# VisionDepth/VisionDepth3D

Hardware: NVIDIA H100
Metric: end-to-end frames/sec (depth+stereo) (higher is better)
Workload: dtype f16 GEMM operands, fp32 accumulate; DIBR fp32

## Files before the change

visiondepth3d_b200/csrc/umma_attention.cuh:

```cuda
#pragma once
#include "umma_gemm.cuh"

namespace vd3d {

struct AttnArgs {
  int ntok;
  int dmodel;
  __half* out;
  int heads;
  int npad;
};

constexpr int kAttnThreads = 384;
constexpr int kAttnKS = 2;
constexpr int kAttnSmem = 16384  + kAttnKS * (16384  + 16384 ) + 1024  + 256 ;

namespace umma {
__device__ __forceinline__ float quad_max(float x) {
  x = fmaxf(x, __shfl_xor_sync(0xffffffffu, x, 1));
  return fmaxf(x, __shfl_xor_sync(0xffffffffu, x, 2));
}
__device__ __forceinline__ float quad_sum(float x) {
  x += __shfl_xor_sync(0xffffffffu, x, 1);
  return x + __shfl_xor_sync(0xffffffffu, x, 2);
}
__device__ __forceinline__ uint32_t pack_h2(float a, float b) {
  __half2 h = __floats2half2_rn(a, b);
  return *(uint32_t*)&h;
}
}

__global__ void __launch_bounds__(kAttnThreads, 1)
k_umma_attention(const __grid_constant__ CUtensorMap tmQ, const __grid_constant__ CUtensorMap tmK,
                 const __grid_constant__ CUtensorMap tmV, const AttnArgs g) {
  extern __shared__ uint8_t smem_raw[];
  const uint32_t sm = (umma::smem_u32(smem_raw) + 1023u) & ~1023u;
  const uint32_t sQ = sm, sK = sm + 16384, sV = sK + kAttnKS * 16384;
  const uint32_t bars = sV + kAttnKS * 16384;
  const uint32_t q_full = bars, kv_full = bars + 8, kv_empty = kv_full + 8 * kAttnKS;

  const int warp = threadIdx.x >> 5, lane = threadIdx.x & 31;
  const int qblk = blockIdx.x, zq = blockIdx.y, h = zq % g.heads, img = zq / g.heads;
  const int T = (g.ntok + 127) / 128;

  if (warp == 0 && lane == 0) {
    umma::prefetch_tmap(&tmQ);
    umma::prefetch_tmap(&tmK);
    umma::prefetch_tmap(&tmV);
    umma::mbar_init(q_full, 1);
    for (int i = 0; i < kAttnKS; ++i) {
      umma::mbar_init(kv_full + 8 * i, 1);
      umma::mbar_init(kv_empty + 8 * i, 2);
    }
    umma::fence_barrier_init();
  }
  __syncthreads();

  if (warp < 4) {
    if (warp == 0 && lane == 0) {
      umma::mbar_expect_tx(q_full, 16384);
      umma::tma_load_3d(sQ, &tmQ, q_full, 0, qblk * 128, zq);
      for (int t = 0; t < T; ++t) {
        const int ks = t % kAttnKS;
        umma::mbar_wait(kv_empty + 8 * ks, ((t / kAttnKS) & 1) ^ 1);
        const uint32_t fb = kv_full + 8 * ks;
        umma::mbar_expect_tx(fb, 32768);
        umma::tma_load_3d(sK + ks * 16384, &tmK, fb, 0, t * 128, zq);
        const uint32_t dst = sV + ks * 16384;
        umma::tma_load_3d(dst, &tmV, fb, t * 128, 0, zq);
        umma::tma_load_3d(dst + 8192, &tmV, fb, t * 128 + 64, 0, zq);
      }
    }
    return;
  }

  const int wg = (warp >> 2) - 1;
  const int wq = warp & 3;
  const float L2E = 1.4426950408889634f;
  const int cq = 2 * (lane & 3);
  float o[32];
#pragma unroll
  for (int i = 0; i < 32; ++i) o[i] = 0.f;
  float m_run[2] = {-INFINITY, -INFINITY}, l_run[2] = {0.f, 0.f};

  umma::mbar_wait(q_full, 0);
  const uint64_t dq = umma::make_desc(sQ + (uint32_t)(wg * 64 * 128));
  for (int t = 0; t < T; ++t) {
    const int ks = t % kAttnKS;
    umma::mbar_wait(kv_full + 8 * ks, (t / kAttnKS) & 1);
    float s[64];
    {
      const uint64_t dk = umma::make_desc(sK + ks * 16384);
      umma::wgmma_fence();
#pragma unroll
      for (int k = 0; k < 4; ++k) umma::wgmma_m64n128_ss(s, dq + (uint64_t)(2 * k), dk + (uint64_t)(2 * k), k ? 1u : 0u);
      umma::wgmma_commit();
      umma::wgmma_wait<0>();
      umma::fence_regs(s);
    }
    const int nvalid = g.ntok - t * 128;
    float mx[2] = {-INFINITY, -INFINITY};
#pragma unroll
    for (int j = 0; j < 16; ++j)
#pragma unroll
      for (int i = 0; i < 4; ++i) {
        if (nvalid < 128 && 8 * j + cq + (i & 1) >= nvalid) s[4 * j + i] = -INFINITY;
        mx[i >> 1] = fmaxf(mx[i >> 1], s[4 * j + i]);
      }
    float scale[2], mref[2];
#pragma unroll
    for (int rr = 0; rr < 2; ++rr) {
      const float m_new = fmaxf(m_run[rr], umma::quad_max(mx[rr]) * L2E);
      scale[rr] = umma::ex2_fast(m_run[rr] - m_new);
      m_run[rr] = m_new;
      mref[rr] = m_new - 8.0f;
    }
    float ls[2] = {0.f, 0.f};
    uint32_t p[32];
#pragma unroll
    for (int j = 0; j < 16; ++j) {
      const float p0 = umma::ex2_fast(fmaf(s[4 * j + 0], L2E, -mref[0]));
      const float p1 = umma::ex2_fast(fmaf(s[4 * j + 1], L2E, -mref[0]));
      const float p2 = umma::ex2_fast(fmaf(s[4 * j + 2], L2E, -mref[1]));
      const float p3 = umma::ex2_fast(fmaf(s[4 * j + 3], L2E, -mref[1]));
      p[2 * j] = umma::pack_h2(p0, p1);
      p[2 * j + 1] = umma::pack_h2(p2, p3);
      const float2 h0 = __half22float2(*(const __half2*)&p[2 * j]), h1 = __half22float2(*(const __half2*)&p[2 * j + 1]);
      ls[0] += h0.x + h0.y;
      ls[1] += h1.x + h1.y;
    }
#pragma unroll
    for (int rr = 0; rr < 2; ++rr) l_run[rr] = l_run[rr] * scale[rr] + ls[rr];
#pragma unroll
    for (int j = 0; j < 8; ++j) {
      o[4 * j + 0] *= scale[0];
      o[4 * j + 1] *= scale[0];
      o[4 * j + 2] *= scale[1];
      o[4 * j + 3] *= scale[1];
    }
    umma::fence_regs(o);
    umma::wgmma_fence();
#pragma unroll
    for (int kk = 0; kk < 8; ++kk) {
      const uint32_t a[4] = {p[4 * kk], p[4 * kk + 1], p[4 * kk + 2], p[4 * kk + 3]};
      const uint64_t db = umma::make_desc(sV + ks * 16384 + (kk >> 2) * 8192) + (uint64_t)(2 * (kk & 3));
      umma::wgmma_m64n64_rs(o, a, db, 1u);
    }
    umma::wgmma_commit();
    umma::wgmma_wait<0>();
    umma::fence_regs(o);
    if ((threadIdx.x & 127) == 0) umma::mbar_arrive(kv_empty + 8 * ks);
  }

  float inv[2];
#pragma unroll
  for (int rr = 0; rr < 2; ++rr) inv[rr] = 1.0f / umma::quad_sum(l_run[rr]);
  const int r0 = qblk * 128 + wg * 64 + wq * 16 + (lane >> 2);
#pragma unroll
  for (int rr = 0; rr < 2; ++rr) {
    const int m = r0 + 8 * rr;
    if (m >= g.ntok) continue;
    __half* dst = g.out + ((size_t)img * g.npad + m) * g.dmodel + h * 64 + cq;
#pragma unroll
    for (int j = 0; j < 8; ++j)
      *(uint32_t*)(dst + 8 * j) = umma::pack_h2(o[4 * j + 2 * rr] * inv[rr], o[4 * j + 2 * rr + 1] * inv[rr]);
  }
}

}
```

Baseline: 320.3.

## Pipeline FA3-style attention with split K/V barriers, ping-pong warpgroups, and register reallocation

```diff
diff --git a/visiondepth3d_b200/csrc/umma_attention.cuh b/visiondepth3d_b200/csrc/umma_attention.cuh
--- a/visiondepth3d_b200/csrc/umma_attention.cuh
+++ b/visiondepth3d_b200/csrc/umma_attention.cuh
@@ -1,4 +1,6 @@
 #pragma once
+#include <type_traits>
+
 #include "umma_gemm.cuh"
 
 namespace vd3d {
@@ -12,8 +14,11 @@
 };
 
 constexpr int kAttnThreads = 384;
-constexpr int kAttnKS = 2;
+constexpr int kAttnKS = 3;
 constexpr int kAttnSmem = 16384  + kAttnKS * (16384  + 16384 ) + 1024  + 256 ;
+constexpr int kAttnProducerRegs = 24;
+constexpr int kAttnConsumerRegs = 240;
+static_assert(128 * kAttnProducerRegs + 256 * kAttnConsumerRegs <= 65536, "register file overcommitted");
 
 namespace umma {
 __device__ __forceinline__ float quad_max(float x) {
@@ -27,6 +32,87 @@
 __device__ __forceinline__ uint32_t pack_h2(float a, float b) {
   __half2 h = __floats2half2_rn(a, b);
   return *(uint32_t*)&h;
+}
+template <int R>
+__device__ __forceinline__ void fence_regs(uint32_t (&d)[R]) {
+#pragma unroll
+  for (int i = 0; i < R; ++i) asm volatile("" : "+r"(d[i])::"memory");
+}
+__device__ __forceinline__ void bar_sync_256(int id) { asm volatile("bar.sync %0, 256;" ::"r"(id) : "memory"); }
+__device__ __forceinline__ void bar_arrive_256(int id) { asm volatile("bar.arrive %0, 256;" ::"r"(id) : "memory"); }
+
+template <bool kMasked>
+__device__ __forceinline__ void attn_softmax(float (&s)[64], int nvalid, int cq, float (&m_run)[2], float (&scale)[2]) {
+  const float L2E = 1.4426950408889634f;
+  if constexpr (kMasked) {
+#pragma unroll
+    for (int j = 0; j < 16; ++j)
+#pragma unroll
+      for (int i = 0; i < 4; ++i)
+        if (8 * j + cq + (i & 1) >= nvalid) s[4 * j + i] = -INFINITY;
+  }
+  float mx[2];
+#pragma unroll
+  for (int rr = 0; rr < 2; ++rr) {
+    float m[16];
+#pragma unroll
+    for (int j = 0; j < 16; ++j) m[j] = fmaxf(s[4 * j + 2 * rr], s[4 * j + 2 * rr + 1]);
+#pragma unroll
+    for (int j = 0; j < 8; ++j) m[j] = fmaxf(m[j], m[j + 8]);
+#pragma unroll
+    for (int j = 0; j < 4; ++j) m[j] = fmaxf(m[j], m[j + 4]);
+    mx[rr] = fmaxf(fmaxf(m[0], m[2]), fmaxf(m[1], m[3]));
+  }
+  float mref[2];
+#pragma unroll
+  for (int rr = 0; rr < 2; ++rr) {
+    const float m_new = fmaxf(m_run[rr], quad_max(mx[rr]) * L2E);
+    scale[rr] = ex2_fast(m_run[rr] - m_new);
+    m_run[rr] = m_new;
+    mref[rr] = m_new - 8.0f;
+  }
+#pragma unroll
+  for (int j = 0; j < 16; ++j)
+#pragma unroll
+    for (int i = 0; i < 4; ++i) s[4 * j + i] = ex2_fast(fmaf(s[4 * j + i], L2E, -mref[i >> 1]));
+}
+
+__device__ __forceinline__ void attn_pack(const float (&s)[64], uint32_t (&p)[32], float (&o)[32], float (&l_run)[2],
+                                          const float (&scale)[2]) {
+  float ls[2] = {0.f, 0.f};
+#pragma unroll
+  for (int j = 0; j < 16; ++j) {
+    p[2 * j] = pack_h2(s[4 * j + 0], s[4 * j + 1]);
+    p[2 * j + 1] = pack_h2(s[4 * j + 2], s[4 * j + 3]);
+    const float2 h0 = __half22float2(*(const __half2*)&p[2 * j]), h1 = __half22float2(*(const __half2*)&p[2 * j + 1]);
+    ls[0] += h0.x + h0.y;
+    ls[1] += h1.x + h1.y;
+  }
+#pragma unroll
+  for (int rr = 0; rr < 2; ++rr) l_run[rr] = l_run[rr] * scale[rr] + ls[rr];
+#pragma unroll
+  for (int j = 0; j < 8; ++j) {
+    o[4 * j + 0] *= scale[0];
+    o[4 * j + 1] *= scale[0];
+    o[4 * j + 2] *= scale[1];
+    o[4 * j + 3] *= scale[1];
+  }
+}
+
+__device__ __forceinline__ void attn_qk(float (&s)[64], uint64_t dq, uint32_t k_tile) {
+  const uint64_t dk = make_desc(k_tile);
+#pragma unroll
+  for (int k = 0; k < 4; ++k) wgmma_m64n128_ss(s, dq + (uint64_t)(2 * k), dk + (uint64_t)(2 * k), k ? 1u : 0u);
+  wgmma_commit();
+}
+__device__ __forceinline__ void attn_pv(float (&o)[32], const uint32_t (&p)[32], uint32_t v_tile) {
+#pragma unroll
+  for (int kk = 0; kk < 8; ++kk) {
+    const uint32_t a[4] = {p[4 * kk], p[4 * kk + 1], p[4 * kk + 2], p[4 * kk + 3]};
+    const uint64_t db = make_desc(v_tile + (kk >> 2) * 8192) + (uint64_t)(2 * (kk & 3));
+    wgmma_m64n64_rs(o, a, db, 1u);
+  }
+  wgmma_commit();
 }
 }
 
@@ -37,7 +123,8 @@
   const uint32_t sm = (umma::smem_u32(smem_raw) + 1023u) & ~1023u;
   const uint32_t sQ = sm, sK = sm + 16384, sV = sK + kAttnKS * 16384;
   const uint32_t bars = sV + kAttnKS * 16384;
-  const uint32_t q_full = bars, kv_full = bars + 8, kv_empty = kv_full + 8 * kAttnKS;
+  const uint32_t q_full = bars, k_full = bars + 8, k_empty = k_full + 8 * kAttnKS;
+  const uint32_t v_full = k_empty + 8 * kAttnKS, v_empty = v_full + 8 * kAttnKS;
 
   const int warp = threadIdx.x >> 5, lane = threadIdx.x & 31;
   const int qblk = blockIdx.x, zq = blockIdx.y, h = zq % g.heads, img = zq / g.heads;
@@ -49,107 +136,96 @@
     umma::prefetch_tmap(&tmV);
     umma::mbar_init(q_full, 1);
     for (int i = 0; i < kAttnKS; ++i) {
-      umma::mbar_init(kv_full + 8 * i, 1);
-      umma::mbar_init(kv_empty + 8 * i, 2);
+      umma::mbar_init(k_full + 8 * i, 1);
+      umma::mbar_init(k_empty + 8 * i, 2);
+      umma::mbar_init(v_full + 8 * i, 1);
+      umma::mbar_init(v_empty + 8 * i, 2);
     }
     umma::fence_barrier_init();
   }
   __syncthreads();
 
   if (warp < 4) {
+    asm volatile("setmaxnreg.dec.sync.aligned.u32 %0;" ::"n"(kAttnProducerRegs));
     if (warp == 0 && lane == 0) {
       umma::mbar_expect_tx(q_full, 16384);
       umma::tma_load_3d(sQ, &tmQ, q_full, 0, qblk * 128, zq);
       for (int t = 0; t < T; ++t) {
         const int ks = t % kAttnKS;
-        umma::mbar_wait(kv_empty + 8 * ks, ((t / kAttnKS) & 1) ^ 1);
-        const uint32_t fb = kv_full + 8 * ks;
-        umma::mbar_expect_tx(fb, 32768);
-        umma::tma_load_3d(sK + ks * 16384, &tmK, fb, 0, t * 128, zq);
-        const uint32_t dst = sV + ks * 16384;
-        umma::tma_load_3d(dst, &tmV, fb, t * 128, 0, zq);
-        umma::tma_load_3d(dst + 8192, &tmV, fb, t * 128 + 64, 0, zq);
+        const uint32_t ph = ((t / kAttnKS) & 1) ^ 1;
+        umma::mbar_wait(k_empty + 8 * ks, ph);
+        umma::mbar_expect_tx(k_full + 8 * ks, 16384);
+        umma::tma_load_3d(sK + ks * 16384, &tmK, k_full + 8 * ks, 0, t * 128, zq);
+        umma::mbar_wait(v_empty + 8 * ks, ph);
+        const uint32_t vb = v_full + 8 * ks, dst = sV + ks * 16384;
+        umma::mbar_expect_tx(vb, 16384);
+        umma::tma_load_3d(dst, &tmV, vb, t * 128, 0, zq);
+        umma::tma_load_3d(dst + 8192, &tmV, vb, t * 128 + 64, 0, zq);
       }
     }
     return;
   }
+  asm volatile("setmaxnreg.inc.sync.aligned.u32 %0;" ::"n"(kAttnConsumerRegs));
 
   const int wg = (warp >> 2) - 1;
   const int wq = warp & 3;
-  const float L2E = 1.4426950408889634f;
   const int cq = 2 * (lane & 3);
+  const bool lead = (threadIdx.x & 127) == 0;
   float o[32];
 #pragma unroll
   for (int i = 0; i < 32; ++i) o[i] = 0.f;
-  float m_run[2] = {-INFINITY, -INFINITY}, l_run[2] = {0.f, 0.f};
+  float m_run[2] = {-INFINITY, -INFINITY}, l_run[2] = {0.f, 0.f}, scale[2];
+  float s[64];
+  uint32_t p[32];
+
+  if (wg == 1) umma::bar_arrive_256(1);
 
   umma::mbar_wait(q_full, 0);
   const uint64_t dq = umma::make_desc(sQ + (uint32_t)(wg * 64 * 128));
-  for (int t = 0; t < T; ++t) {
-    const int ks = t % kAttnKS;
-    umma::mbar_wait(kv_full + 8 * ks, (t / kAttnKS) & 1);
-    float s[64];
-    {
-      const uint64_t dk = umma::make_desc(sK + ks * 16384);
-      umma::wgmma_fence();
-#pragma unroll
-      for (int k = 0; k < 4; ++k) umma::wgmma_m64n128_ss(s, dq + (uint64_t)(2 * k), dk + (uint64_t)(2 * k), k ? 1u : 0u);
-      umma::wgmma_commit();
-      umma::wgmma_wait<0>();
-      umma::fence_regs(s);
-    }
-    const int nvalid = g.ntok - t * 128;
-    float mx[2] = {-INFINITY, -INFINITY};
-#pragma unroll
-    for (int j = 0; j < 16; ++j)
-#pragma unroll
-      for (int i = 0; i < 4; ++i) {
-        if (nvalid < 128 && 8 * j + cq + (i & 1) >= nvalid) s[4 * j + i] = -INFINITY;
-        mx[i >> 1] = fmaxf(mx[i >> 1], s[4 * j + i]);
-      }
-    float scale[2], mref[2];
-#pragma unroll
-    for (int rr = 0; rr < 2; ++rr) {
-      const float m_new = fmaxf(m_run[rr], umma::quad_max(mx[rr]) * L2E);
-      scale[rr] = umma::ex2_fast(m_run[rr] - m_new);
-      m_run[rr] = m_new;
-      mref[rr] = m_new - 8.0f;
-    }
-    float ls[2] = {0.f, 0.f};
-    uint32_t p[32];
-#pragma unroll
-    for (int j = 0; j < 16; ++j) {
-      const float p0 = umma::ex2_fast(fmaf(s[4 * j + 0], L2E, -mref[0]));
-      const float p1 = umma::ex2_fast(fmaf(s[4 * j + 1], L2E, -mref[0]));
-      const float p2 = umma::ex2_fast(fmaf(s[4 * j + 2], L2E, -mref[1]));
-      const float p3 = umma::ex2_fast(fmaf(s[4 * j + 3], L2E, -mref[1]));
-      p[2 * j] = umma::pack_h2(p0, p1);
-      p[2 * j + 1] = umma::pack_h2(p2, p3);
-      const float2 h0 = __half22float2(*(const __half2*)&p[2 * j]), h1 = __half22float2(*(const __half2*)&p[2 * j + 1]);
-      ls[0] += h0.x + h0.y;
-      ls[1] += h1.x + h1.y;
-    }
-#pragma unroll
-    for (int rr = 0; rr < 2; ++rr) l_run[rr] = l_run[rr] * scale[rr] + ls[rr];
-#pragma unroll
-    for (int j = 0; j < 8; ++j) {
-      o[4 * j + 0] *= scale[0];
-      o[4 * j + 1] *= scale[0];
-      o[4 * j + 2] *= scale[1];
-      o[4 * j + 3] *= scale[1];
-    }
+  umma::mbar_wait(k_full, 0);
+  umma::bar_sync_256(1 + wg);
+  umma::wgmma_fence();
+  umma::attn_qk(s, dq, sK);
+  umma::bar_arrive_256(2 - wg);
+  umma::wgmma_wait<0>();
+  umma::fence_regs(s);
+  if (lead) umma::mbar_arrive(k_empty);
+  umma::attn_softmax<true>(s, g.ntok, cq, m_run, scale);
+  umma::attn_pack(s, p, o, l_run, scale);
+
+  auto round = [&](int t, auto masked) {
+    const int ks = t % kAttnKS, vs = (t - 1) % kAttnKS;
+    umma::mbar_wait(k_full + 8 * ks, (t / kAttnKS) & 1);
+    umma::mbar_wait(v_full + 8 * vs, ((t - 1) / kAttnKS) & 1);
+    umma::bar_sync_256(1 + wg);
     umma::fence_regs(o);
     umma::wgmma_fence();
-#pragma unroll
-    for (int kk = 0; kk < 8; ++kk) {
-      const uint32_t a[4] = {p[4 * kk], p[4 * kk + 1], p[4 * kk + 2], p[4 * kk + 3]};
-      const uint64_t db = umma::make_desc(sV + ks * 16384 + (kk >> 2) * 8192) + (uint64_t)(2 * (kk & 3));
-      umma::wgmma_m64n64_rs(o, a, db, 1u);
-    }
-    umma::wgmma_commit();
+    umma::attn_qk(s, dq, sK + ks * 16384);
+    umma::attn_pv(o, p, sV + vs * 16384);
+    umma::bar_arrive_256(2 - wg);
+    umma::wgmma_wait<1>();
+    umma::fence_regs(s);
+    if (lead) umma::mbar_arrive(k_empty + 8 * ks);
+    umma::attn_softmax<decltype(masked)::value>(s, g.ntok - t * 128, cq, m_run, scale);
     umma::wgmma_wait<0>();
     umma::fence_regs(o);
-    if ((threadIdx.x & 127) == 0) umma::mbar_arrive(kv_empty + 8 * ks);
+    umma::fence_regs(p);
+    if (lead) umma::mbar_arrive(v_empty + 8 * vs);
+    umma::attn_pack(s, p, o, l_run, scale);
+  };
+  for (int t = 1; t < T - 1; ++t) round(t, std::false_type{});
+  if (T > 1) round(T - 1, std::true_type{});
+
+  {
+    const int vs = (T - 1) % kAttnKS;
+    umma::mbar_wait(v_full + 8 * vs, ((T - 1) / kAttnKS) & 1);
+    umma::bar_sync_256(1 + wg);
+    umma::fence_regs(o);
+    umma::wgmma_fence();
+    umma::attn_pv(o, p, sV + vs * 16384);
+    if (wg == 0) umma::bar_arrive_256(2);
+    umma::wgmma_wait<0>();
+    umma::fence_regs(o);
   }
 
   float inv[2];
```

After: 327.7, median of 6. +2.3%, better.
